# evalf/nutils

Hardware: AMD Instinct MI355X
Metric: elements assembled/sec (global stiffness K) (higher is better)
Workload: dtype f64; 1 GPU; 3D Poisson stiffness, 128^3 structured hex, p=1, 2x2x2 Gauss, iso geometry (BASELINE.json configs[1]); nelems_per_gpu=2097152, nnz_per_gpu=57066625, kernel=k_p1hex_skew<16,16,false,false>, parallelism=single GPU, launch=hipGraph replay (20 steps per graph), settle_steps=600

## Files before the change

nutils_amd/csrc/nh_assemble_p1hex.hip:

```cpp
#include "nh_common.h"
#include <algorithm>
#include <type_traits>
#include <cstdio>
#include <cstdlib>

namespace {

#ifdef NH_ABLATION
#define DEBUG(p) ((p).debug)
#else
#define DEBUG(p) 0
#endif

struct P1Args {
  int n0, n1, n2;
  int lay0, lay1;
  int pl0, pl1;
  const double *verts;
  double origin[3], scale[3];
  double n[2][2];
  double c[3][2];
  double wk[2][2][2];
  double wm[2][2][2];
  int hasm;
  const double *qmass;
  double *values;
  const double *qscale;
  const double *u;
  double *out;
  int accumulate;
  int nbj, nbk;
  long long *tdbg;
  int wbnd;
  int debug;
};

__device__ __forceinline__ int len_of(int X, int N) { return (X > 0) + 1 + (X < N - 1); }
__device__ __forceinline__ i64 cum_of(int X, int N) { return X == 0 ? 0 : 3 * (i64)X - 1; }

__device__ __forceinline__ double fast_rcp(double d) {
  double r = __builtin_amdgcn_rcp(d);
  r = fma(fma(-d, r, 1.), r, r);
  r = fma(fma(-d, r, 1.), r, r);
  return r;
}

__device__ __forceinline__ void lds_barrier() { asm volatile("s_waitcnt lgkmcnt(0)\n\ts_barrier" ::: "memory"); }

struct ElemTables {
  double R0[3][3], R1[3][3], R2[3][3];
  double W01[2][2][3], W02[2][2][3], W12[2][2][3];
  double Mm[3][3][3];
};

__device__ __forceinline__ double element_entry(const ElemTables &T, int a, int bb) {
  const int a0 = a >> 2, a1 = (a >> 1) & 1, a2 = a & 1;
// ... 288 lines not shown
}
__device__ __forceinline__ void half_wait(unsigned *cnt, unsigned target) {
  while (__hip_atomic_load(cnt, __ATOMIC_RELAXED, __HIP_MEMORY_SCOPE_WORKGROUP) < target) __builtin_amdgcn_s_sleep(1);
  asm volatile("" ::: "memory");
}

template <int TJ, int TK, bool MASS, bool COEF>
__global__ __launch_bounds__(2 * TJ * TK) void k_p1hex_skew(P1Args p) {
  constexpr bool VEC = false;
#ifdef NH_ABLATION
  long long tacc[10] = {0, 0, 0, 0, 0, 0, 0, 0, 0, 0}, tprev = clock64();
  const long long tstart = tprev;
  int nslow = 0, nfast = 0;
#ifdef NH_NOTICKS
#define NH_TICK(i)
#else
#define NH_TICK(i) { const long long tnow = clock64(); tacc[i] += tnow - tprev; tprev = tnow; }
#endif
#else
#define NH_TICK(i)
#endif
  constexpr int G = TJ * TK, NT = 2 * G, NP = 4, OJ = TJ - 1, OK = TK - 1, NS = 15, VW = 3;
  constexpr int VJ = TJ + 1, VK = TK + 1, RP = VJ * VK, PS = (RP * NS + 1) & ~1, VPG = (RP + G - 1) / G;
  const bool getenv_stage_late = p.wbnd < 0;
  extern __shared__ __attribute__((aligned(16))) double lds[];
  double *acc = lds;
  double *vbuf = lds + NP * PS;
  unsigned *hcnt = reinterpret_cast<unsigned *>(vbuf + 3 * RP * VW);
  const int tid = threadIdx.x, lt = tid & (G - 1), grp = __builtin_amdgcn_readfirstlane(tid / G);
  const int N0 = p.n0 + 1, N1 = p.n1 + 1, N2 = p.n2 + 1;
  const int NPL = p.pl1 - p.pl0;
  const unsigned wg = gridDim.x % 8 == 0 ? (blockIdx.x % 8) * (gridDim.x / 8) + blockIdx.x / 8 : blockIdx.x;
  const i64 CP = NPL + 2, WI = 16, WB = p.nbj > 1 ? (p.wbnd < 0 ? -p.wbnd : p.wbnd) : 16;
  const i64 rowB = p.nbk * CP * WB, rowI = p.nbk * CP * WI, nmid = max(p.nbj - 2, 0);
  const i64 ctot = (p.nbj > 1 ? 2 : 1) * rowB + nmid * rowI;
  auto unit_at = [&](i64 c) {
    i64 jt, rem, w;
    if (c < rowB) jt = 0, rem = c, w = WB;
    else if (c < rowB + nmid * rowI) jt = 1 + (c - rowB) / rowI, rem = (c - rowB) % rowI, w = WI;
    else jt = p.nbj > 1 ? p.nbj - 1 : 1, rem = c - rowB - nmid * rowI, w = WB;
    const i64 kt = rem / (CP * w), pos = (rem - kt * CP * w) / w;
    return (jt * p.nbk + kt) * NPL + min(max(pos - 1, (i64)0), (i64)NPL);
  };
  i64 u = unit_at(ctot * wg / gridDim.x);
  const i64 u1 = unit_at(ctot * (wg + 1) / gridDim.x);
  if (u >= u1) return;
  auto slot_of = [](int P) { return (int)((unsigned)(P + 2 * NP) % NP) * PS; };
  auto vslot_of = [](int P) { return (int)((unsigned)(P + 3) % 3) * (RP * VW); };
  auto load_vertex = [&](int I, int r, int J0, int K0, double (&x)[3]) {
    const int bb = r / VK, c = r % VK, J = J0 - 1 + bb, K = K0 - 1 + c;
    x[0] = x[1] = x[2] = 0.;
    if (r < RP && I >= 0 && I < N0 && J >= 0 && J < N1 && K >= 0 && K < N2) {
      const double *src = p.verts + (((i64)I * N1 + J) * N2 + K) * 3;
      x[0] = src[0], x[1] = src[1], x[2] = src[2];
    }
  };
  if (tid == 0) *hcnt = 0;
  unsigned htarget = 0;
  const i64 T1 = 3 * (i64)N1 - 2, T2 = 3 * (i64)N2 - 2;
  while (u < u1) {
    const int col = (int)(u / NPL), A = p.pl0 + (int)(u % NPL), B = (int)min((i64)p.pl1, A + (u1 - u));
    const int J0 = (col / p.nbk) * OJ, K0 = (col % p.nbk) * OK;
    {
      constexpr int NVL = (2 * RP + NT - 1) / NT;
      double x[NVL][3];
      bool valid[NVL];
#pragma unroll
      for (int k = 0; k < NVL; ++k) {
        const int v = min(tid + k * NT, 2 * RP - 1), pl = v / RP, r = v % RP, I = A - 1 + pl;
        const int J = J0 - 1 + r / VK, K = K0 - 1 + r % VK;
        valid[k] = I >= 0 && I < N0 && J >= 0 && J < N1 && K >= 0 && K < N2;
        const double *src = p.verts + (((i64)min(max(I, 0), N0 - 1) * N1 + min(max(J, 0), N1 - 1)) * N2 + min(max(K, 0), N2 - 1)) * 3;
        x[k][0] = src[0], x[k][1] = src[1], x[k][2] = src[2];
      }
      for (int t = tid; t < NP * PS / 2; t += NT) reinterpret_cast<double2 *>(acc)[t] = make_double2(0., 0.);
#pragma unroll
      for (int k = 0; k < NVL; ++k) {
        const int v = tid + k * NT, pl = v / RP, r = v % RP;
        if (v < 2 * RP) {
          double *dst = vbuf + vslot_of(A - 1 + pl) + r * VW;
          dst[0] = valid[k] ? x[k][0] : 0., dst[1] = valid[k] ? x[k][1] : 0., dst[2] = valid[k] ? x[k][2] : 0.;
        }
      }
    }
    lds_barrier();

    for (int s = A - 1; s <= B; ++s) {
      htarget += G / 64;
      NH_TICK(0)
      const bool mathrole = ((s - (A - 1)) & 1) == grp;
      if (mathrole) {
        const int ej = lt / TK, ek = lt % TK;
        const int gi = s, gj = J0 - 1 + ej, gk = K0 - 1 + ek;
        if (s < B && gi >= p.lay0 && gi < p.lay1 && gj >= 0 && gj < p.n1 && gk >= 0 && gk < p.n2 && !(DEBUG(p) & 4)) {
#define NH_P1HEX_VERT(a, bb, c) (vbuf + vslot_of(gi + (a)) + ((ej + (bb)) * VK + (ek + (c))) * VW)
#include "nh_p1hex_element.inc"
#undef NH_P1HEX_VERT
        }
        NH_TICK(3)
      } else {
        const bool needv = s + 1 < B && !(DEBUG(p) & 8);
        double Vn[VPG][3];
#pragma unroll
        for (int k = 0; k < VPG; ++k) load_vertex(needv ? s + 2 : -1, lt + k * G, J0, K0, Vn[k]);
        const int P = s - 1;
        bool arrived = false, staged = false;
        auto stage_vertices = [&]() {
#pragma unroll
          for (int k = 0; k < VPG; ++k) {
            const int r = lt + k * G;
            if (r < RP) {
              double *dst = vbuf + vslot_of(s + 2) + r * VW;
              dst[0] = Vn[k][0], dst[1] = Vn[k][1], dst[2] = Vn[k][2];
            }
          }
        };
        if (P >= A && !(DEBUG(p) & 2)) {
          const bool lowJ = J0 == 0, highJ = J0 + OJ >= N1;
          const int cumJ0 = J0 == 0 ? 0 : 3 * J0 - 1;
#ifdef NH_ABLATION
          if (!lowJ && !highJ && P > 0 && P < N0 - 1 && K0 > 0 && K0 + OK < N2) ++nfast; else ++nslow;
#endif
          if (!lowJ && !highJ && P > 0 && P < N0 - 1 && K0 > 0 && K0 + OK < N2) {
            const int e = 2 * lt;
            auto source = [&](int ee, bool &below) {
              const int ok_ = ee / 27, sl_ = ee - ok_ * 27;
              const int dJ_ = (sl_ / 3) % 3 - 1, dK_ = sl_ % 3 - 1;
              below = sl_ < 9;
              return (VK + ok_ + 1) * NS + (sl_ >= 13 ? sl_ - 13 : (dJ_ * VK + dK_) * NS + 13 - sl_);
            };
            bool belowA, belowB;
            const int offA = source(e < 405 ? e : 404, belowA), offB = source(e + 1 < 405 ? e + 1 : 404, belowB);
            const double *sA = acc + (belowA ? slot_of(P - 1) : slot_of(P)) + offA;
            const double *sB = acc + (belowB ? slot_of(P - 1) : slot_of(P)) + offB;
            double a0[OJ], a1[OJ];
#pragma unroll
            for (int i = 0; i < OJ; ++i) {
              a0[i] = sA[i * (VK * NS)];
              a1[i] = sB[i * (VK * NS)];
            }
            const int li = lt - 202;
            const bool lone = li >= 0 && li < OJ;
            bool belowL;
            const int offL = source(404, belowL);
            const double aL = acc[(belowL ? slot_of(P - 1) : slot_of(P)) + offL + (lone ? li : 0) * (VK * NS)];
            half_arrive(hcnt);
            arrived = true;
            NH_TICK(8)
            if (needv && !getenv_stage_late) {
              __builtin_amdgcn_s_waitcnt(0x0f70);
              stage_vertices();
              staged = true;
            }
            const i64 stride8 = 8 * (i64)(9 * (int)T2);
            char *l0 = reinterpret_cast<char *>(p.values + ((3 * (i64)P - 1) * T1 * T2 + 3 * (cumJ0 * T2) + 9 * (3 * (i64)K0 - 1)));
            char *lp = l0 + 16 * lt;
            if (lt < 202) {
#pragma unroll
              for (int i = 0; i < OJ; ++i) {
                if ((DEBUG(p) & 16) && (i & 1)) continue;
                const double2 v = make_double2(a0[i], a1[i]);
                __builtin_memcpy(lp + i * stride8, &v, 16);
              }
            }
            if (lone) *reinterpret_cast<double *>(l0 + li * stride8 + 8 * 404) = aL;
          } else {
            constexpr int RPP = G / 32, KP = (OK + RPP - 1) / RPP;
            const int sl = lt & 31, rsub = lt >> 5;
            const int dI = sl / 9 - 1, dJ = (sl / 3) % 3 - 1, dK = sl % 3 - 1;
            const bool upper = sl >= 13;
            const int need = (dI < 0 ? 1 : dI > 0 ? 8 : 0) | (dJ < 0 ? 2 : dJ > 0 ? 16 : 0) | (dK < 0 ? 4 : dK > 0 ? 32 : 0);
            const int loI = P > 0, hiI = P < N0 - 1, lenI = loI + 1 + hiI;
            double v[KP][OJ];
#pragma unroll
            for (int kp = 0; kp < KP; ++kp) {
              const int ok = kp * RPP + rsub;
              const int srow = (VK + ok + 1) * NS + (upper ? sl - 13 : (dJ * VK + dK) * NS + 13 - sl);
              const double *src = acc + ((!upper && dI < 0) ? slot_of(P - 1) : slot_of(P)) + (ok < OK ? srow : 0);
#pragma unroll
              for (int oj = 0; oj < OJ; ++oj) v[kp][oj] = src[oj * (VK * NS)];
            }
            half_arrive(hcnt);
            arrived = true;
#pragma unroll
            for (int kp = 0; kp < KP; ++kp) {
              const int ok = kp * RPP + rsub, Kk = K0 + ok;
              const bool kact = sl < 27 && ok < OK && Kk < N2;
              const int loK = Kk > 0, hiK = Kk < N2 - 1, lenK = loK + 1 + hiK, cumK = Kk == 0 ? 0 : 3 * Kk - 1;
              double *line = p.values + ((P == 0 ? 0 : 3 * (i64)P - 1) * T1 * T2 + lenI * (cumJ0 * T2));
              if (!lowJ && !highJ) {
                const int flag = loI | 2 | loK << 2 | hiI << 3 | 16 | hiK << 5;
                const unsigned voff8 = 8u * (unsigned)(lenI * 3 * cumK + ((dI + loI) * 3 + (dJ + 1)) * lenK + (dK + loK));
                const i64 stride8 = 8 * (i64)(lenI * 3 * (int)T2);
                if (kact && (flag & need) == need) {
                  char *lp = reinterpret_cast<char *>(line);
#pragma unroll
                  for (int oj = 0; oj < OJ; ++oj) {
                    if (!((DEBUG(p) & 16) && (oj & 1))) *reinterpret_cast<double *>(lp + voff8) = v[kp][oj];
                    lp += stride8;
                  }
                }
              } else {
#pragma unroll
                for (int oj = 0; oj < OJ; ++oj) {
                  const int J = J0 + oj;
                  const int loJ = J > 0, hiJ = J < N1 - 1, lenJ = loJ + 1 + hiJ;
                  const int flag = loI | loJ << 1 | loK << 2 | hiI << 3 | hiJ << 4 | hiK << 5;
                  const unsigned voff = (unsigned)(lenI * lenJ * cumK + ((dI + loI) * lenJ + (dJ + loJ)) * lenK + (dK + loK));
                  if (kact && J < N1 && (flag & need) == need && !((DEBUG(p) & 16) && (oj & 1))) line[voff] = v[kp][oj];
                  line += lenI * lenJ * (int)T2;
                }
              }
            }
          }
        }
        NH_TICK(6)
        if (!arrived) half_arrive(hcnt);
        half_wait(hcnt, htarget);
        NH_TICK(7)
        {
          double2 *z = reinterpret_cast<double2 *>(acc + slot_of(s - 2));
          for (int t = lt; t < PS / 2; t += G) z[t] = make_double2(0., 0.);
        }
        NH_TICK(9)
        if (needv && !staged) stage_vertices();
      }
      if (mathrole) { NH_TICK(1) } else { NH_TICK(4) }
      lds_barrier();
      if (mathrole) { NH_TICK(2) } else { NH_TICK(5) }
    }
    u += B - A;
  }
#ifdef NH_ABLATION
  if (p.tdbg && tid == 0) {
    p.tdbg[16 + 4 * blockIdx.x] = clock64() - tstart;
    p.tdbg[16 + 4 * blockIdx.x + 1] = nfast;
    p.tdbg[16 + 4 * blockIdx.x + 2] = nslow;
  }
  if (p.tdbg && (tid & 63) == 0)
    for (int i = 0; i < 10; ++i) atomicAdd((unsigned long long *)p.tdbg + i, (unsigned long long)tacc[i]);
#endif
}
#undef NH_TICK

__global__ void k_p1hex_unit_matrix(P1Args p, double *Ke) {
  double X[2][2][2][3];
  for (int a = 0; a < 2; ++a)
    for (int b = 0; b < 2; ++b)
      for (int c = 0; c < 2; ++c) {
        X[a][b][c][0] = p.origin[0] + p.scale[0] * a;
        X[a][b][c][1] = p.origin[1] + p.scale[1] * b;
        X[a][b][c][2] = p.origin[2] + p.scale[2] * c;
      }
  ElemTables T;
  {
    double (&R0)[3][3] = T.R0, (&R1)[3][3] = T.R1, (&R2)[3][3] = T.R2;
    double (&W01)[2][2][3] = T.W01, (&W02)[2][2][3] = T.W02, (&W12)[2][2][3] = T.W12;
    double (&Mm)[3][3][3] = T.Mm;
    for (int i = 0; i < 27; ++i) (&Mm[0][0][0])[i] = 0.;
    const bool hasm = p.hasm;
#define NH_P1HEX_QS(q) 1.
#define NH_P1HEX_QM(q) 1.
#include "nh_p1hex_math.inc"
// ... 81 lines not shown
    if (r >= (i64)N0 * N1 * N2) return (3 * (i64)N0 - 2) * T1 * T2;
    const int Kk = (int)(r % N2), J = (int)((r / N2) % N1), I = (int)(r / ((i64)N2 * N1));
    return cum_of(I, N0) * T1 * T2 + len_of(I, N0) * (cum_of(J, N1) * T2 + (i64)len_of(J, N1) * cum_of(Kk, N2));
  };
  const i64 base = rp(row0);
  if (slot == 0) rowptr[row - row0] = rp(row) - base;
  if (row >= row1) return;
  const int Kk = (int)(row % N2), J = (int)((row / N2) % N1), I = (int)(row / ((i64)N2 * N1));
  const int dI = slot / 9 - 1, dJ = (slot / 3) % 3 - 1, dK = slot % 3 - 1;
  const int cI = I + dI, cJ = J + dJ, cK = Kk + dK;
  if (cI < 0 || cI >= N0 || cJ < 0 || cJ >= N1 || cK < 0 || cK >= N2) return;
  const int lenJ = len_of(J, N1), lenK = len_of(Kk, N2);
  const int pos = ((dI + (I > 0)) * lenJ + (dJ + (J > 0))) * lenK + (dK + (Kk > 0));
  colidx[rp(row) - base + pos] = ((i64)cI * N1 + cJ) * N2 + cK;
}

}

template <bool VEC, bool MASS, bool COEF>
static int launch_march_inst(const nh_p1hex_args *a, P1Args &p, void *stream) {
#ifdef NH_ABLATION
  p.debug = getenv("NH_P1HEX_DEBUG") ? atoi(getenv("NH_P1HEX_DEBUG")) : 0;
#endif
  p.wbnd = 20;
#ifdef NH_ABLATION
  static const int wbnd_env = getenv("NH_P1HEX_WBND") ? std::min(64, std::max(8, atoi(getenv("NH_P1HEX_WBND")))) : 20;
  p.wbnd = getenv("NH_P1HEX_STAGE_LATE") ? -wbnd_env : wbnd_env;
#endif
  constexpr int TJ = 16, TK = 16, L = 2, NTM = L * TJ * TK, NS = VEC ? 1 : 15, VW = VEC ? 4 : 3;
  int dev = 0;
  NH_CHECK_HIP(hipGetDevice(&dev));
  NH_REQUIRE(dev >= 0 && dev < 16, "nh_p1hex: device index %d not supported", dev);
  static int cus_of[16] = {0};
  if (!cus_of[dev]) {
    int n = 256;
    NH_CHECK_HIP(hipDeviceGetAttribute(&n, hipDeviceAttributeMultiprocessorCount, dev));
    cus_of[dev] = n;
  }
  const int cus = cus_of[dev];
  p.nbj = (p.n1 + 1 + TJ - 2) / (TJ - 1);
  p.nbk = (p.n2 + 1 + TK - 2) / (TK - 1);
  const size_t ldsm = sizeof(double) * ((L + 2) * (((TJ + 1) * (TK + 1) * NS + 1) & ~1) + (L + 1) * (TJ + 1) * (TK + 1) * VW + 2);
  const i64 units = (i64)p.nbj * p.nbk * (p.pl1 - p.pl0);
  NH_REQUIRE(a->max_workgroups >= 0, "nh_p1hex: negative max_workgroups");
  unsigned grid = (unsigned)std::min<i64>(units, a->max_workgroups ? std::min(cus, a->max_workgroups) : cus);
#ifdef NH_ABLATION
  if (getenv("NH_P1HEX_MAXWG")) grid = std::min<unsigned>(grid, (unsigned)atoi(getenv("NH_P1HEX_MAXWG")));
#endif
  auto kern = k_p1hex_march<TJ, TK, L, VEC, MASS, COEF>;
  if constexpr (!VEC && L == 2) {
    const char *env = getenv("NH_P1HEX_KERNEL");
    if (!(env && !strcmp(env, "march"))) kern = k_p1hex_skew<TJ, TK, MASS, COEF>;
  }
  static const void *attr_set[16][2] = {{nullptr, nullptr}};
  if (attr_set[dev][0] != (const void *)kern && attr_set[dev][1] != (const void *)kern) {
    NH_CHECK_HIP(hipFuncSetAttribute((const void *)kern, hipFuncAttributeMaxDynamicSharedMemorySize, (int)ldsm));
    attr_set[dev][attr_set[dev][0] ? 1 : 0] = (const void *)kern;
  }
#ifdef NH_ABLATION
  static long long *tdbg = nullptr;
  if (!tdbg) NH_CHECK_HIP(hipMalloc((void **)&tdbg, (16 + 4 * 1024) * sizeof(long long)));
  NH_CHECK_HIP(hipMemsetAsync(tdbg, 0, (16 + 4 * 1024) * sizeof(long long), nh_stream(stream)));
  p.tdbg = getenv("NH_P1HEX_TIMERS") ? tdbg : nullptr;
#endif
  hipLaunchKernelGGL(kern, dim3(grid), dim3(NTM), ldsm, nh_stream(stream), p);
  NH_LAUNCH_CHECK();
#ifdef NH_ABLATION
  if (p.tdbg) {
    static long long h[16 + 4 * 1024];
    NH_CHECK_HIP(hipMemcpy(h, tdbg, sizeof h, hipMemcpyDeviceToHost));
    if (getenv("NH_P1HEX_WGTIMES"))
      for (unsigned g = 0; g < grid; ++g) fprintf(stderr, "wg %u cycles %lld fast %lld slow %lld\n", g, h[16 + 4 * g], h[16 + 4 * g + 1], h[16 + 4 * g + 2]);
    const double nw = (double)grid * (NTM / 64);
    if (kern != (void (*)(P1Args))k_p1hex_march<TJ, TK, L, VEC, MASS, COEF>)
      fprintf(stderr, "p1hex_skew cycles per wave: prologue %.0f | math %.0f | - %.0f | math wait %.0f | lds reads %.0f | store issue %.0f | half wait %.0f | zero %.0f | stage %.0f | mem wait %.0f\n", h[0] / nw, h[3] / nw, h[1] / nw,
              h[2] / nw, h[8] / nw, h[6] / nw, h[7] / nw, h[9] / nw, h[4] / nw, h[5] / nw);
    else
    fprintf(stderr, "p1hex_march cycles per wave: stage+next %.0f | B1 %.0f | load+math %.0f | B2 %.0f | stage+flush %.0f | B3 %.0f | zero %.0f\n", h[0] / nw, h[1] / nw,
            h[2] / nw, h[3] / nw, h[4] / nw, h[5] / nw, h[6] / nw);
  }
#endif
  return NH_OK;
}

template <bool VEC>
static int launch_march(const nh_p1hex_args *a, P1Args &p, void *stream) {
  const bool coef = p.qscale || p.qmass;
  if (p.hasm) return coef ? launch_march_inst<VEC, true, true>(a, p, stream) : launch_march_inst<VEC, true, false>(a, p, stream);
  return coef ? launch_march_inst<VEC, false, true>(a, p, stream) : launch_march_inst<VEC, false, false>(a, p, stream);
}

extern "C" {

int nh_p1hex_pattern(const int *shape, int64_t row_begin, int64_t row_end, int64_t *rowptr_dev, int64_t *colidx_dev, void *stream) {
  NH_REQUIRE(shape && rowptr_dev && colidx_dev, "nh_p1hex_pattern: NULL argument");
  NH_REQUIRE(shape[0] >= 1 && shape[1] >= 1 && shape[2] >= 1, "nh_p1hex_pattern: empty mesh");
  const i64 nrows_total = (i64)(shape[0] + 1) * (shape[1] + 1) * (shape[2] + 1);
  NH_REQUIRE(0 <= row_begin && row_begin <= row_end && row_end <= nrows_total, "nh_p1hex_pattern: row range out of bounds");
  const i64 n = (row_end - row_begin + 1) * 27;
  hipLaunchKernelGGL(k_p1hex_pattern, dim3((unsigned)((n + 255) / 256)), dim3(256), 0, nh_stream(stream), shape[0], shape[1], shape[2],
// ... 22 lines not shown
  }
  for (int q = 0; q < 2; ++q) {
    p.n[0][q] = 1. - a->gauss_x[q];
    p.n[1][q] = a->gauss_x[q];
    p.c[0][q] = p.n[0][q] * p.n[0][q];
    p.c[1][q] = p.n[0][q] * p.n[1][q];
    p.c[2][q] = p.n[1][q] * p.n[1][q];
  }
  for (int qa = 0; qa < 2; ++qa)
    for (int qb = 0; qb < 2; ++qb)
      for (int qc = 0; qc < 2; ++qc) {
        p.wk[qa][qb][qc] = a->kappa * a->gauss_w[qa] * a->gauss_w[qb] * a->gauss_w[qc];
        p.wm[qa][qb][qc] = a->mass * a->gauss_w[qa] * a->gauss_w[qb] * a->gauss_w[qc];
      }
  p.hasm = a->mass != 0. || a->qmass_dev != nullptr;
  p.qmass = a->qmass_dev;
  p.values = a->values_dev;
  p.qscale = a->qscale_dev;
  p.u = nullptr;
  p.out = nullptr;
  p.accumulate = 0;
  p.nbj = p.nbk = 0;
  p.debug = 0;
  p.wbnd = 16;
  p.tdbg = nullptr;
  return NH_OK;
}

int nh_p1hex_unit_matrix(const nh_p1hex_args *a, double *ke_dev, void *stream) {
  NH_REQUIRE(ke_dev, "nh_p1hex_unit_matrix: NULL output");
  P1Args p;
  int rc = fill_p1args(a, p);
  if (rc) return rc;
  hipLaunchKernelGGL(k_p1hex_unit_matrix, dim3(1), dim3(1), 0, nh_stream(stream), p, ke_dev);
  NH_LAUNCH_CHECK();
  return NH_OK;
}

int nh_p1hex_laplace(const nh_p1hex_args *a, void *stream) {
  NH_REQUIRE(a && a->values_dev, "nh_p1hex_laplace: NULL argument");
  P1Args p;
  int rc = fill_p1args(a, p);
  if (rc) return rc;
  if (a->plane_begin == a->plane_end) return NH_OK;
  NH_REQUIRE(!(a->qscale_dev || a->qmass_dev) || a->verts_dev, "nh_p1hex_laplace: a coefficient array needs explicit vertices");
  if (!a->verts_dev) {
    double *Ke = nullptr;
// ... 28 lines not shown
```

Before: 12.31 billion elements/s.

## Split workgroups into interior and boundary classes with specialized kernel bodies

Work partitioning now puts boundary column tiles and interior column tiles into separate workgroup classes. Separate weights for the low and high boundary rows and for the corner tiles balance the load between them. The kernel body moves into an include that is instantiated twice. The interior-only version drops the boundary checks and the slow scatter path, and the boundary version adds extra stores for the J-boundary rows. This aims to cut branch and bookkeeping overhead in the common interior case and to improve load balance, at the cost of more code, more register pressure and new host-side split logic.

```diff
diff --git a/nutils_amd/csrc/nh_assemble_p1hex.hip b/nutils_amd/csrc/nh_assemble_p1hex.hip
--- a/nutils_amd/csrc/nh_assemble_p1hex.hip
+++ b/nutils_amd/csrc/nh_assemble_p1hex.hip
@@ -1,4 +1,5 @@
 #include "nh_common.h"
+#include "nh_p1hex_split.h"
 #include <algorithm>
 #include <type_traits>
 #include <cstdio>
@@ -10,6 +11,19 @@
 #define DEBUG(p) ((p).debug)
 #else
 #define DEBUG(p) 0
+#endif
+
+#ifndef NH_P1HEX_WLOW_DEFAULT
+#define NH_P1HEX_WLOW_DEFAULT 19
+#endif
+#ifndef NH_P1HEX_WHIGH_DEFAULT
+#define NH_P1HEX_WHIGH_DEFAULT 18
+#endif
+#ifndef NH_P1HEX_WCLOW_DEFAULT
+#define NH_P1HEX_WCLOW_DEFAULT 22
+#endif
+#ifndef NH_P1HEX_WCHIGH_DEFAULT
+#define NH_P1HEX_WCHIGH_DEFAULT 24
 #endif
 
 struct P1Args {
@@ -31,7 +45,9 @@
   int accumulate;
   int nbj, nbk;
   long long *tdbg;
-  int wbnd;
+  int gb, nfront;
+  int wclow, wchigh;
+  int wlow, whigh;
   int debug;
 };
 
@@ -366,7 +382,7 @@
 #endif
   constexpr int G = TJ * TK, NT = 2 * G, NP = 4, OJ = TJ - 1, OK = TK - 1, NS = 15, VW = 3;
   constexpr int VJ = TJ + 1, VK = TK + 1, RP = VJ * VK, PS = (RP * NS + 1) & ~1, VPG = (RP + G - 1) / G;
-  const bool getenv_stage_late = p.wbnd < 0;
+  const bool getenv_stage_late = p.wlow < 0;
   extern __shared__ __attribute__((aligned(16))) double lds[];
   double *acc = lds;
   double *vbuf = lds + NP * PS;
@@ -375,20 +391,11 @@
   const int N0 = p.n0 + 1, N1 = p.n1 + 1, N2 = p.n2 + 1;
   const int NPL = p.pl1 - p.pl0;
   const unsigned wg = gridDim.x % 8 == 0 ? (blockIdx.x % 8) * (gridDim.x / 8) + blockIdx.x / 8 : blockIdx.x;
-  const i64 CP = NPL + 2, WI = 16, WB = p.nbj > 1 ? (p.wbnd < 0 ? -p.wbnd : p.wbnd) : 16;
-  const i64 rowB = p.nbk * CP * WB, rowI = p.nbk * CP * WI, nmid = max(p.nbj - 2, 0);
-  const i64 ctot = (p.nbj > 1 ? 2 : 1) * rowB + nmid * rowI;
-  auto unit_at = [&](i64 c) {
-    i64 jt, rem, w;
-    if (c < rowB) jt = 0, rem = c, w = WB;
-    else if (c < rowB + nmid * rowI) jt = 1 + (c - rowB) / rowI, rem = (c - rowB) % rowI, w = WI;
-    else jt = p.nbj > 1 ? p.nbj - 1 : 1, rem = c - rowB - nmid * rowI, w = WB;
-    const i64 kt = rem / (CP * w), pos = (rem - kt * CP * w) / w;
-    return (jt * p.nbk + kt) * NPL + min(max(pos - 1, (i64)0), (i64)NPL);
-  };
-  i64 u = unit_at(ctot * wg / gridDim.x);
-  const i64 u1 = unit_at(ctot * (wg + 1) / gridDim.x);
-  if (u >= u1) return;
+  const P1SplitGeom geom = {p.nbj, p.nbk, NPL, p.wlow < 0 ? -p.wlow : p.wlow, p.whigh, p.wclow, p.wchigh};
+  auto uniform = [](i64 x) { return (i64)(((unsigned long long)(unsigned)__builtin_amdgcn_readfirstlane((int)(x >> 32)) << 32) | (unsigned)__builtin_amdgcn_readfirstlane((int)x)); };
+  P1Split sp = nh_p1hex_split_share(geom, gridDim.x, wg, p.gb, p.nfront);
+  sp.cls = __builtin_amdgcn_readfirstlane(sp.cls), sp.v0 = uniform(sp.v0), sp.v1 = uniform(sp.v1);
+  if (sp.v0 >= sp.v1) return;
   auto slot_of = [](int P) { return (int)((unsigned)(P + 2 * NP) % NP) * PS; };
   auto vslot_of = [](int P) { return (int)((unsigned)(P + 3) % 3) * (RP * VW); };
   auto load_vertex = [&](int I, int r, int J0, int K0, double (&x)[3]) {
@@ -402,187 +409,24 @@
   if (tid == 0) *hcnt = 0;
   unsigned htarget = 0;
   const i64 T1 = 3 * (i64)N1 - 2, T2 = 3 * (i64)N2 - 2;
-  while (u < u1) {
-    const int col = (int)(u / NPL), A = p.pl0 + (int)(u % NPL), B = (int)min((i64)p.pl1, A + (u1 - u));
-    const int J0 = (col / p.nbk) * OJ, K0 = (col % p.nbk) * OK;
-    {
-      constexpr int NVL = (2 * RP + NT - 1) / NT;
-      double x[NVL][3];
-      bool valid[NVL];
-#pragma unroll
-      for (int k = 0; k < NVL; ++k) {
-        const int v = min(tid + k * NT, 2 * RP - 1), pl = v / RP, r = v % RP, I = A - 1 + pl;
-        const int J = J0 - 1 + r / VK, K = K0 - 1 + r % VK;
-        valid[k] = I >= 0 && I < N0 && J >= 0 && J < N1 && K >= 0 && K < N2;
-        const double *src = p.verts + (((i64)min(max(I, 0), N0 - 1) * N1 + min(max(J, 0), N1 - 1)) * N2 + min(max(K, 0), N2 - 1)) * 3;
-        x[k][0] = src[0], x[k][1] = src[1], x[k][2] = src[2];
-      }
-      for (int t = tid; t < NP * PS / 2; t += NT) reinterpret_cast<double2 *>(acc)[t] = make_double2(0., 0.);
-#pragma unroll
-      for (int k = 0; k < NVL; ++k) {
-        const int v = tid + k * NT, pl = v / RP, r = v % RP;
-        if (v < 2 * RP) {
-          double *dst = vbuf + vslot_of(A - 1 + pl) + r * VW;
-          dst[0] = valid[k] ? x[k][0] : 0., dst[1] = valid[k] ? x[k][1] : 0., dst[2] = valid[k] ? x[k][2] : 0.;
-        }
-      }
-    }
-    lds_barrier();
-
-    for (int s = A - 1; s <= B; ++s) {
-      htarget += G / 64;
-      NH_TICK(0)
-      const bool mathrole = ((s - (A - 1)) & 1) == grp;
-      if (mathrole) {
-        const int ej = lt / TK, ek = lt % TK;
-        const int gi = s, gj = J0 - 1 + ej, gk = K0 - 1 + ek;
-        if (s < B && gi >= p.lay0 && gi < p.lay1 && gj >= 0 && gj < p.n1 && gk >= 0 && gk < p.n2 && !(DEBUG(p) & 4)) {
-#define NH_P1HEX_VERT(a, bb, c) (vbuf + vslot_of(gi + (a)) + ((ej + (bb)) * VK + (ek + (c))) * VW)
-#include "nh_p1hex_element.inc"
-#undef NH_P1HEX_VERT
-        }
-        NH_TICK(3)
-      } else {
-        const bool needv = s + 1 < B && !(DEBUG(p) & 8);
-        double Vn[VPG][3];
-#pragma unroll
-        for (int k = 0; k < VPG; ++k) load_vertex(needv ? s + 2 : -1, lt + k * G, J0, K0, Vn[k]);
-        const int P = s - 1;
-        bool arrived = false, staged = false;
-        auto stage_vertices = [&]() {
-#pragma unroll
-          for (int k = 0; k < VPG; ++k) {
-            const int r = lt + k * G;
-            if (r < RP) {
-              double *dst = vbuf + vslot_of(s + 2) + r * VW;
-              dst[0] = Vn[k][0], dst[1] = Vn[k][1], dst[2] = Vn[k][2];
-            }
-          }
-        };
-        if (P >= A && !(DEBUG(p) & 2)) {
-          const bool lowJ = J0 == 0, highJ = J0 + OJ >= N1;
-          const int cumJ0 = J0 == 0 ? 0 : 3 * J0 - 1;
-#ifdef NH_ABLATION
-          if (!lowJ && !highJ && P > 0 && P < N0 - 1 && K0 > 0 && K0 + OK < N2) ++nfast; else ++nslow;
-#endif
-          if (!lowJ && !highJ && P > 0 && P < N0 - 1 && K0 > 0 && K0 + OK < N2) {
-            const int e = 2 * lt;
-            auto source = [&](int ee, bool &below) {
-              const int ok_ = ee / 27, sl_ = ee - ok_ * 27;
-              const int dJ_ = (sl_ / 3) % 3 - 1, dK_ = sl_ % 3 - 1;
-              below = sl_ < 9;
-              return (VK + ok_ + 1) * NS + (sl_ >= 13 ? sl_ - 13 : (dJ_ * VK + dK_) * NS + 13 - sl_);
-            };
-            bool belowA, belowB;
-            const int offA = source(e < 405 ? e : 404, belowA), offB = source(e + 1 < 405 ? e + 1 : 404, belowB);
-            const double *sA = acc + (belowA ? slot_of(P - 1) : slot_of(P)) + offA;
-            const double *sB = acc + (belowB ? slot_of(P - 1) : slot_of(P)) + offB;
-            double a0[OJ], a1[OJ];
-#pragma unroll
-            for (int i = 0; i < OJ; ++i) {
-              a0[i] = sA[i * (VK * NS)];
-              a1[i] = sB[i * (VK * NS)];
-            }
-            const int li = lt - 202;
-            const bool lone = li >= 0 && li < OJ;
-            bool belowL;
-            const int offL = source(404, belowL);
-            const double aL = acc[(belowL ? slot_of(P - 1) : slot_of(P)) + offL + (lone ? li : 0) * (VK * NS)];
-            half_arrive(hcnt);
-            arrived = true;
-            NH_TICK(8)
-            if (needv && !getenv_stage_late) {
-              __builtin_amdgcn_s_waitcnt(0x0f70);
-              stage_vertices();
-              staged = true;
-            }
-            const i64 stride8 = 8 * (i64)(9 * (int)T2);
-            char *l0 = reinterpret_cast<char *>(p.values + ((3 * (i64)P - 1) * T1 * T2 + 3 * (cumJ0 * T2) + 9 * (3 * (i64)K0 - 1)));
-            char *lp = l0 + 16 * lt;
-            if (lt < 202) {
-#pragma unroll
-              for (int i = 0; i < OJ; ++i) {
-                if ((DEBUG(p) & 16) && (i & 1)) continue;
-                const double2 v = make_double2(a0[i], a1[i]);
-                __builtin_memcpy(lp + i * stride8, &v, 16);
-              }
-            }
-            if (lone) *reinterpret_cast<double *>(l0 + li * stride8 + 8 * 404) = aL;
-          } else {
-            constexpr int RPP = G / 32, KP = (OK + RPP - 1) / RPP;
-            const int sl = lt & 31, rsub = lt >> 5;
-            const int dI = sl / 9 - 1, dJ = (sl / 3) % 3 - 1, dK = sl % 3 - 1;
-            const bool upper = sl >= 13;
-            const int need = (dI < 0 ? 1 : dI > 0 ? 8 : 0) | (dJ < 0 ? 2 : dJ > 0 ? 16 : 0) | (dK < 0 ? 4 : dK > 0 ? 32 : 0);
-            const int loI = P > 0, hiI = P < N0 - 1, lenI = loI + 1 + hiI;
-            double v[KP][OJ];
-#pragma unroll
-            for (int kp = 0; kp < KP; ++kp) {
-              const int ok = kp * RPP + rsub;
-              const int srow = (VK + ok + 1) * NS + (upper ? sl - 13 : (dJ * VK + dK) * NS + 13 - sl);
-              const double *src = acc + ((!upper && dI < 0) ? slot_of(P - 1) : slot_of(P)) + (ok < OK ? srow : 0);
-#pragma unroll
-              for (int oj = 0; oj < OJ; ++oj) v[kp][oj] = src[oj * (VK * NS)];
-            }
-            half_arrive(hcnt);
-            arrived = true;
-#pragma unroll
-            for (int kp = 0; kp < KP; ++kp) {
-              const int ok = kp * RPP + rsub, Kk = K0 + ok;
-              const bool kact = sl < 27 && ok < OK && Kk < N2;
-              const int loK = Kk > 0, hiK = Kk < N2 - 1, lenK = loK + 1 + hiK, cumK = Kk == 0 ? 0 : 3 * Kk - 1;
-              double *line = p.values + ((P == 0 ? 0 : 3 * (i64)P - 1) * T1 * T2 + lenI * (cumJ0 * T2));
-              if (!lowJ && !highJ) {
-                const int flag = loI | 2 | loK << 2 | hiI << 3 | 16 | hiK << 5;
-                const unsigned voff8 = 8u * (unsigned)(lenI * 3 * cumK + ((dI + loI) * 3 + (dJ + 1)) * lenK + (dK + loK));
-                const i64 stride8 = 8 * (i64)(lenI * 3 * (int)T2);
-                if (kact && (flag & need) == need) {
-                  char *lp = reinterpret_cast<char *>(line);
-#pragma unroll
-                  for (int oj = 0; oj < OJ; ++oj) {
-                    if (!((DEBUG(p) & 16) && (oj & 1))) *reinterpret_cast<double *>(lp + voff8) = v[kp][oj];
-                    lp += stride8;
-                  }
-                }
-              } else {
-#pragma unroll
-                for (int oj = 0; oj < OJ; ++oj) {
-                  const int J = J0 + oj;
-                  const int loJ = J > 0, hiJ = J < N1 - 1, lenJ = loJ + 1 + hiJ;
-                  const int flag = loI | loJ << 1 | loK << 2 | hiI << 3 | hiJ << 4 | hiK << 5;
-                  const unsigned voff = (unsigned)(lenI * lenJ * cumK + ((dI + loI) * lenJ + (dJ + loJ)) * lenK + (dK + loK));
-                  if (kact && J < N1 && (flag & need) == need && !((DEBUG(p) & 16) && (oj & 1))) line[voff] = v[kp][oj];
-                  line += lenI * lenJ * (int)T2;
-                }
-              }
-            }
-          }
-        }
-        NH_TICK(6)
-        if (!arrived) half_arrive(hcnt);
-        half_wait(hcnt, htarget);
-        NH_TICK(7)
-        {
-          double2 *z = reinterpret_cast<double2 *>(acc + slot_of(s - 2));
-          for (int t = lt; t < PS / 2; t += G) z[t] = make_double2(0., 0.);
-        }
-        NH_TICK(9)
-        if (needv && !staged) stage_vertices();
-      }
-      if (mathrole) { NH_TICK(1) } else { NH_TICK(4) }
-      lds_barrier();
-      if (mathrole) { NH_TICK(2) } else { NH_TICK(5) }
-    }
-    u += B - A;
+  if (!MASS && !COEF && sp.cls == NH_P1_INTERIOR) {
+#define NH_P1HEX_BND false
+#include "nh_p1hex_skew_run.inc"
+#undef NH_P1HEX_BND
+  } else {
+#define NH_P1HEX_BND true
+#include "nh_p1hex_skew_run.inc"
+#undef NH_P1HEX_BND
   }
 #ifdef NH_ABLATION
   if (p.tdbg && tid == 0) {
-    p.tdbg[16 + 4 * blockIdx.x] = clock64() - tstart;
-    p.tdbg[16 + 4 * blockIdx.x + 1] = nfast;
-    p.tdbg[16 + 4 * blockIdx.x + 2] = nslow;
+    p.tdbg[32 + 4 * blockIdx.x] = clock64() - tstart;
+    p.tdbg[32 + 4 * blockIdx.x + 1] = nfast;
+    p.tdbg[32 + 4 * blockIdx.x + 2] = nslow;
+    p.tdbg[32 + 4 * blockIdx.x + 3] = sp.cls;
   }
   if (p.tdbg && (tid & 63) == 0)
-    for (int i = 0; i < 10; ++i) atomicAdd((unsigned long long *)p.tdbg + i, (unsigned long long)tacc[i]);
+    for (int i = 0; i < 10; ++i) atomicAdd((unsigned long long *)p.tdbg + (sp.cls == NH_P1_INTERIOR ? 0 : 10) + i, (unsigned long long)tacc[i]);
 #endif
 }
 #undef NH_TICK
@@ -710,10 +554,16 @@
 #ifdef NH_ABLATION
   p.debug = getenv("NH_P1HEX_DEBUG") ? atoi(getenv("NH_P1HEX_DEBUG")) : 0;
 #endif
-  p.wbnd = 20;
-#ifdef NH_ABLATION
-  static const int wbnd_env = getenv("NH_P1HEX_WBND") ? std::min(64, std::max(8, atoi(getenv("NH_P1HEX_WBND")))) : 20;
-  p.wbnd = getenv("NH_P1HEX_STAGE_LATE") ? -wbnd_env : wbnd_env;
+  p.wlow = NH_P1HEX_WLOW_DEFAULT;
+  p.whigh = NH_P1HEX_WHIGH_DEFAULT;
+  p.wclow = NH_P1HEX_WCLOW_DEFAULT;
+  p.wchigh = NH_P1HEX_WCHIGH_DEFAULT;
+#ifdef NH_ABLATION
+  if (getenv("NH_P1HEX_WLOW")) p.wlow = std::min(64, std::max(8, atoi(getenv("NH_P1HEX_WLOW"))));
+  if (getenv("NH_P1HEX_WHIGH")) p.whigh = std::min(64, std::max(8, atoi(getenv("NH_P1HEX_WHIGH"))));
+  if (getenv("NH_P1HEX_WCLOW")) p.wclow = std::min(64, std::max(8, atoi(getenv("NH_P1HEX_WCLOW"))));
+  if (getenv("NH_P1HEX_WCHIGH")) p.wchigh = std::min(64, std::max(8, atoi(getenv("NH_P1HEX_WCHIGH"))));
+  if (getenv("NH_P1HEX_STAGE_LATE")) p.wlow = -p.wlow;
 #endif
   constexpr int TJ = 16, TK = 16, L = 2, NTM = L * TJ * TK, NS = VEC ? 1 : 15, VW = VEC ? 4 : 3;
   int dev = 0;
@@ -747,23 +597,47 @@
   }
 #ifdef NH_ABLATION
   static long long *tdbg = nullptr;
-  if (!tdbg) NH_CHECK_HIP(hipMalloc((void **)&tdbg, (16 + 4 * 1024) * sizeof(long long)));
-  NH_CHECK_HIP(hipMemsetAsync(tdbg, 0, (16 + 4 * 1024) * sizeof(long long), nh_stream(stream)));
+  if (!tdbg) NH_CHECK_HIP(hipMalloc((void **)&tdbg, (32 + 4 * 1024) * sizeof(long long)));
+  NH_CHECK_HIP(hipMemsetAsync(tdbg, 0, (32 + 4 * 1024) * sizeof(long long), nh_stream(stream)));
   p.tdbg = getenv("NH_P1HEX_TIMERS") ? tdbg : nullptr;
 #endif
+  {
+    const P1SplitGeom geom = {p.nbj, p.nbk, p.pl1 - p.pl0, p.wlow < 0 ? -p.wlow : p.wlow, p.whigh, p.wclow, p.wchigh};
+    const P1SplitClasses c = nh_p1hex_split_classes(geom, grid);
+    p.gb = (int)c.gb, p.nfront = (int)c.nfront;
+  }
   hipLaunchKernelGGL(kern, dim3(grid), dim3(NTM), ldsm, nh_stream(stream), p);
   NH_LAUNCH_CHECK();
 #ifdef NH_ABLATION
   if (p.tdbg) {
-    static long long h[16 + 4 * 1024];
+    static long long h[32 + 4 * 1024];
     NH_CHECK_HIP(hipMemcpy(h, tdbg, sizeof h, hipMemcpyDeviceToHost));
-    if (getenv("NH_P1HEX_WGTIMES"))
-      for (unsigned g = 0; g < grid; ++g) fprintf(stderr, "wg %u cycles %lld fast %lld slow %lld\n", g, h[16 + 4 * g], h[16 + 4 * g + 1], h[16 + 4 * g + 2]);
     const double nw = (double)grid * (NTM / 64);
-    if (kern != (void (*)(P1Args))k_p1hex_march<TJ, TK, L, VEC, MASS, COEF>)
-      fprintf(stderr, "p1hex_skew cycles per wave: prologue %.0f | math %.0f | - %.0f | math wait %.0f | lds reads %.0f | store issue %.0f | half wait %.0f | zero %.0f | stage %.0f | mem wait %.0f\n", h[0] / nw, h[3] / nw, h[1] / nw,
-              h[2] / nw, h[8] / nw, h[6] / nw, h[7] / nw, h[9] / nw, h[4] / nw, h[5] / nw);
-    else
+    if (kern != (void (*)(P1Args))k_p1hex_march<TJ, TK, L, VEC, MASS, COEF>) {
+      static const char *const cname[3] = {"interior", "boundary", "mixed"};
+      double cnt[3] = {0, 0, 0}, sum[3] = {0, 0, 0}, lo[3] = {0, 0, 0}, hi[3] = {0, 0, 0};
+      for (unsigned g = 0; g < grid; ++g) {
+        const long long cyc = h[32 + 4 * g], c = std::min(2ll, std::max(0ll, h[32 + 4 * g + 3]));
+        if (!cyc) continue;
+        if (getenv("NH_P1HEX_WGTIMES")) {
+          const P1SplitGeom geom = {p.nbj, p.nbk, p.pl1 - p.pl0, p.wlow < 0 ? -p.wlow : p.wlow, p.whigh, p.wclow, p.wchigh};
+          const unsigned share = grid % 8 == 0 ? (g % 8) * (grid / 8) + g / 8 : g;
+          const P1Split s = nh_p1hex_split(geom, grid, share);
+          const long long col = nh_p1hex_class_column(geom, s.cls, s.v0 / geom.npl);
+          fprintf(stderr, "wg %u share %u class %s first column jt %lld kt %lld units %lld cycles %lld fast %lld slow %lld\n", g, share, cname[c], col / p.nbk, col % p.nbk, s.v1 - s.v0, cyc,
+                  h[32 + 4 * g + 1], h[32 + 4 * g + 2]);
+        }
+        lo[c] = cnt[c] ? std::min(lo[c], (double)cyc) : (double)cyc, hi[c] = std::max(hi[c], (double)cyc), sum[c] += cyc, cnt[c] += 1;
+      }
+      for (int c = 0; c < 3; ++c)
+        if (cnt[c]) fprintf(stderr, "p1hex_skew class %s: %.0f workgroups, cycles mean %.0f min %.0f max %.0f\n", cname[c], cnt[c], sum[c] / cnt[c], lo[c], hi[c]);
+      for (int b = 0; b < 2; ++b) {
+        const double nwb = (b ? cnt[1] + cnt[2] : cnt[0]) * (NTM / 64);
+        const long long *t = h + 10 * b;
+        if (nwb) fprintf(stderr, "p1hex_skew %s body, cycles per wave: prologue %.0f | math %.0f | - %.0f | math wait %.0f | lds reads %.0f | store issue %.0f | half wait %.0f | zero %.0f | stage %.0f | mem wait %.0f\n",
+                         b ? "boundary" : "interior", t[0] / nwb, t[3] / nwb, t[1] / nwb, t[2] / nwb, t[8] / nwb, t[6] / nwb, t[7] / nwb, t[9] / nwb, t[4] / nwb, t[5] / nwb);
+      }
+    } else
     fprintf(stderr, "p1hex_march cycles per wave: stage+next %.0f | B1 %.0f | load+math %.0f | B2 %.0f | stage+flush %.0f | B3 %.0f | zero %.0f\n", h[0] / nw, h[1] / nw,
             h[2] / nw, h[3] / nw, h[4] / nw, h[5] / nw, h[6] / nw);
   }
@@ -832,7 +706,8 @@
   p.accumulate = 0;
   p.nbj = p.nbk = 0;
   p.debug = 0;
-  p.wbnd = 16;
+  p.wlow = p.whigh = p.wclow = p.wchigh = 16;
+  p.gb = p.nfront = 0;
   p.tdbg = nullptr;
   return NH_OK;
 }
diff --git a/nutils_amd/csrc/nh_p1hex_skew_run.inc b/nutils_amd/csrc/nh_p1hex_skew_run.inc
--- /dev/null
+++ b/nutils_amd/csrc/nh_p1hex_skew_run.inc
@@ -0,0 +1,212 @@
+{
+  constexpr bool BND = NH_P1HEX_BND;
+  int tid_ = tid, lt_ = lt;
+  asm volatile("" : "+v"(tid_), "+v"(lt_));
+  {
+  const int tid = tid_ & (NT - 1), lt = lt_ & (G - 1);
+  i64 u = sp.v0;
+  const i64 u1 = sp.v1;
+  while (u < u1) {
+    const int col = __builtin_amdgcn_readfirstlane((int)nh_p1hex_class_column(geom, BND ? sp.cls : NH_P1_INTERIOR, u / NPL)), A = __builtin_amdgcn_readfirstlane(p.pl0 + (int)(u % NPL));
+    const int B = (int)min((i64)p.pl1, A + (u1 - u));
+    const int J0 = (col / p.nbk) * OJ, K0 = (col % p.nbk) * OK;
+    {
+      constexpr int NVL = (2 * RP + NT - 1) / NT;
+      double x[NVL][3];
+      bool valid[NVL];
+#pragma unroll
+      for (int k = 0; k < NVL; ++k) {
+        const int v = min(tid + k * NT, 2 * RP - 1), pl = v / RP, r = v % RP, I = A - 1 + pl;
+        const int J = J0 - 1 + r / VK, K = K0 - 1 + r % VK;
+        valid[k] = I >= 0 && I < N0 && J >= 0 && J < N1 && K >= 0 && K < N2;
+        const double *src = p.verts + (((i64)min(max(I, 0), N0 - 1) * N1 + min(max(J, 0), N1 - 1)) * N2 + min(max(K, 0), N2 - 1)) * 3;
+        x[k][0] = src[0], x[k][1] = src[1], x[k][2] = src[2];
+      }
+      for (int t = tid; t < NP * PS / 2; t += NT) reinterpret_cast<double2 *>(acc)[t] = make_double2(0., 0.);
+#pragma unroll
+      for (int k = 0; k < NVL; ++k) {
+        const int v = tid + k * NT, pl = v / RP, r = v % RP;
+        if (v < 2 * RP) {
+          double *dst = vbuf + vslot_of(A - 1 + pl) + r * VW;
+          dst[0] = valid[k] ? x[k][0] : 0., dst[1] = valid[k] ? x[k][1] : 0., dst[2] = valid[k] ? x[k][2] : 0.;
+        }
+      }
+    }
+    lds_barrier();
+
+    for (int s = A - 1; s <= B; ++s) {
+      htarget += G / 64;
+      NH_TICK(0)
+      const bool mathrole = ((s - (A - 1)) & 1) == grp;
+      if (mathrole) {
+        const int ej = lt / TK, ek = lt % TK;
+        const int gi = s, gj = J0 - 1 + ej, gk = K0 - 1 + ek;
+        if (s < B && gi >= p.lay0 && gi < p.lay1 && gj >= 0 && gj < p.n1 && gk >= 0 && gk < p.n2 && !(DEBUG(p) & 4)) {
+#define NH_P1HEX_VERT(a, bb, c) (vbuf + vslot_of(gi + (a)) + ((ej + (bb)) * VK + (ek + (c))) * VW)
+#include "nh_p1hex_element.inc"
+#undef NH_P1HEX_VERT
+        }
+        NH_TICK(3)
+      } else {
+        const bool needv = s + 1 < B && !(DEBUG(p) & 8);
+        double Vn[VPG][3];
+#pragma unroll
+        for (int k = 0; k < VPG; ++k) load_vertex(needv ? s + 2 : -1, lt + k * G, J0, K0, Vn[k]);
+        const int P = s - 1;
+        bool arrived = false, staged = false;
+        auto stage_vertices = [&]() {
+#pragma unroll
+          for (int k = 0; k < VPG; ++k) {
+            const int r = lt + k * G;
+            if (r < RP) {
+              double *dst = vbuf + vslot_of(s + 2) + r * VW;
+              dst[0] = Vn[k][0], dst[1] = Vn[k][1], dst[2] = Vn[k][2];
+            }
+          }
+        };
+        if (P >= A && !(DEBUG(p) & 2)) {
+          const bool lowJ = BND && J0 == 0, highJ = BND && J0 + OJ >= N1;
+          const int cumJ0 = 3 * J0 - 1;
+          const bool linewise = !(lowJ && highJ) && P > 0 && P < N0 - 1 && K0 > 0 && K0 + OK < N2;
+#ifdef NH_ABLATION
+          if (linewise) ++nfast; else ++nslow;
+#endif
+          if (linewise) {
+            const int jlo = lowJ ? 1 : 0, jhi = highJ ? N1 - 1 - J0 : OJ;
+            const int e = 2 * lt;
+            auto source = [&](int ee, bool &below) {
+              const int ok_ = ee / 27, sl_ = ee - ok_ * 27;
+              const int dJ_ = (sl_ / 3) % 3 - 1, dK_ = sl_ % 3 - 1;
+              below = sl_ < 9;
+              return (VK + ok_ + 1) * NS + (sl_ >= 13 ? sl_ - 13 : (dJ_ * VK + dK_) * NS + 13 - sl_);
+            };
+            bool belowA, belowB;
+            const int offA = source(e < 405 ? e : 404, belowA), offB = source(e + 1 < 405 ? e + 1 : 404, belowB);
+            const double *sA = acc + (belowA ? slot_of(P - 1) : slot_of(P)) + offA;
+            const double *sB = acc + (belowB ? slot_of(P - 1) : slot_of(P)) + offB;
+            double a0[OJ], a1[OJ];
+#pragma unroll
+            for (int i = 0; i < OJ; ++i) {
+              if (!BND || (i >= jlo && i < jhi)) {
+                a0[i] = sA[i * (VK * NS)];
+                a1[i] = sB[i * (VK * NS)];
+              } else a0[i] = a1[i] = 0.;
+            }
+            const int li = lt - 202;
+            const bool lone = li >= jlo && li < jhi;
+            bool belowL;
+            const int offL = source(404, belowL);
+            const double aL = acc[(belowL ? slot_of(P - 1) : slot_of(P)) + offL + (lone ? li : jlo < jhi ? jlo : 0) * (VK * NS)];
+            double b0 = 0., b1 = 0.;
+            if (BND && (lowJ || highJ) && lt < 135) {
+              int e = 2 * lt;
+              asm volatile("" : "+v"(e));
+              const int jb = lowJ ? 0 : N1 - 1 - J0;
+              auto source18 = [&](int ee, bool &below) {
+                const int ok_ = ee / 18, s_ = ee - ok_ * 18;
+                const int dJ_ = (s_ / 3) % 2 - (lowJ ? 0 : 1), dK_ = s_ % 3 - 1, sl_ = (s_ / 6) * 9 + (dJ_ + 1) * 3 + (dK_ + 1);
+                below = sl_ < 9;
+                return (VK + ok_ + 1) * NS + (sl_ >= 13 ? sl_ - 13 : (dJ_ * VK + dK_) * NS + 13 - sl_);
+              };
+              bool belowC, belowD;
+              const int offC = source18(e, belowC) + jb * (VK * NS), offD = source18(e + 1, belowD) + jb * (VK * NS);
+              b0 = acc[(belowC ? slot_of(P - 1) : slot_of(P)) + offC];
+              b1 = acc[(belowD ? slot_of(P - 1) : slot_of(P)) + offD];
+            }
+            half_arrive(hcnt);
+            arrived = true;
+            NH_TICK(8)
+            if (needv && !getenv_stage_late) {
+              __builtin_amdgcn_s_waitcnt(0x0f70);
+              stage_vertices();
+              staged = true;
+            }
+            const i64 stride8 = 8 * (i64)(9 * (int)T2);
+            char *const pbase = reinterpret_cast<char *>(p.values + (3 * (i64)P - 1) * T1 * T2);
+            char *l0 = pbase + 8 * (3 * (cumJ0 * T2) + 9 * (3 * (i64)K0 - 1));
+            char *lp = l0 + 16 * lt;
+            if (lt < 202) {
+#pragma unroll
+              for (int i = 0; i < OJ; ++i) {
+                if ((DEBUG(p) & 16) && (i & 1)) continue;
+                if (BND && !(i >= jlo && i < jhi)) continue;
+                const double2 v = make_double2(a0[i], a1[i]);
+                __builtin_memcpy(lp + i * stride8, &v, 16);
+              }
+            }
+            if (lone) *reinterpret_cast<double *>(l0 + li * stride8 + 8 * 404) = aL;
+            if (BND && (lowJ || highJ) && lt < 135) {
+              const i64 cumJb = lowJ ? 0 : 3 * (i64)(N1 - 1) - 1;
+              const double2 v = make_double2(b0, b1);
+              __builtin_memcpy(pbase + 8 * (3 * (cumJb * T2) + 6 * (3 * (i64)K0 - 1)) + 16 * lt, &v, 16);
+            }
+          } else {
+            constexpr int RPP = G / 32, KP = (OK + RPP - 1) / RPP;
+            const int sl = lt & 31, rsub = lt >> 5;
+            const int dI = sl / 9 - 1, dJ = (sl / 3) % 3 - 1, dK = sl % 3 - 1;
+            const bool upper = sl >= 13;
+            const int need = (dI < 0 ? 1 : dI > 0 ? 8 : 0) | (dJ < 0 ? 2 : dJ > 0 ? 16 : 0) | (dK < 0 ? 4 : dK > 0 ? 32 : 0);
+            const int loI = P > 0, hiI = P < N0 - 1, lenI = loI + 1 + hiI;
+            const int cumJ0g = J0 == 0 ? 0 : cumJ0;
+            double v[KP][OJ];
+#pragma unroll
+            for (int kp = 0; kp < KP; ++kp) {
+              const int ok = kp * RPP + rsub;
+              const int srow = (VK + ok + 1) * NS + (upper ? sl - 13 : (dJ * VK + dK) * NS + 13 - sl);
+              const double *src = acc + ((!upper && dI < 0) ? slot_of(P - 1) : slot_of(P)) + (ok < OK ? srow : 0);
+#pragma unroll
+              for (int oj = 0; oj < OJ; ++oj) v[kp][oj] = src[oj * (VK * NS)];
+            }
+            half_arrive(hcnt);
+            arrived = true;
+#pragma unroll
+            for (int kp = 0; kp < KP; ++kp) {
+              const int ok = kp * RPP + rsub, Kk = K0 + ok;
+              const bool kact = sl < 27 && ok < OK && Kk < N2;
+              const int loK = Kk > 0, hiK = Kk < N2 - 1, lenK = loK + 1 + hiK, cumK = Kk == 0 ? 0 : 3 * Kk - 1;
+              double *line = p.values + ((P == 0 ? 0 : 3 * (i64)P - 1) * T1 * T2 + lenI * (cumJ0g * T2));
+              if (!lowJ && !highJ) {
+                const int flag = loI | 2 | loK << 2 | hiI << 3 | 16 | hiK << 5;
+                const unsigned voff8 = 8u * (unsigned)(lenI * 3 * cumK + ((dI + loI) * 3 + (dJ + 1)) * lenK + (dK + loK));
+                const i64 stride8 = 8 * (i64)(lenI * 3 * (int)T2);
+                if (kact && (flag & need) == need) {
+                  char *lp = reinterpret_cast<char *>(line);
+#pragma unroll
+                  for (int oj = 0; oj < OJ; ++oj) {
+                    if (!((DEBUG(p) & 16) && (oj & 1))) *reinterpret_cast<double *>(lp + voff8) = v[kp][oj];
+                    lp += stride8;
+                  }
+                }
+              } else {
+#pragma unroll
+                for (int oj = 0; oj < OJ; ++oj) {
+                  const int J = J0 + oj;
+                  const int loJ = J > 0, hiJ = J < N1 - 1, lenJ = loJ + 1 + hiJ;
+                  const int flag = loI | loJ << 1 | loK << 2 | hiI << 3 | hiJ << 4 | hiK << 5;
+                  const unsigned voff = (unsigned)(lenI * lenJ * cumK + ((dI + loI) * lenJ + (dJ + loJ)) * lenK + (dK + loK));
+                  if (kact && J < N1 && (flag & need) == need && !((DEBUG(p) & 16) && (oj & 1))) line[voff] = v[kp][oj];
+                  line += lenI * lenJ * (int)T2;
+                }
+              }
+            }
+          }
+        }
+        NH_TICK(6)
+        if (!arrived) half_arrive(hcnt);
+        half_wait(hcnt, htarget);
+        NH_TICK(7)
+        {
+          double2 *z = reinterpret_cast<double2 *>(acc + slot_of(s - 2));
+          for (int t = lt; t < PS / 2; t += G) z[t] = make_double2(0., 0.);
+        }
+        NH_TICK(9)
+        if (needv && !staged) stage_vertices();
+      }
+      if (mathrole) { NH_TICK(1) } else { NH_TICK(4) }
+      lds_barrier();
+      if (mathrole) { NH_TICK(2) } else { NH_TICK(5) }
+    }
+    u += B - A;
+  }
+  }
+}
diff --git a/nutils_amd/csrc/nh_p1hex_split.h b/nutils_amd/csrc/nh_p1hex_split.h
--- /dev/null
+++ b/nutils_amd/csrc/nh_p1hex_split.h
@@ -0,0 +1,107 @@
+#ifndef NH_P1HEX_SPLIT_H
+#define NH_P1HEX_SPLIT_H
+
+#if defined(__HIPCC__)
+#define NH_SPLIT_FN __host__ __device__ __attribute__((always_inline)) inline
+#else
+#define NH_SPLIT_FN inline
+#endif
+
+enum { NH_P1_INTERIOR = 0, NH_P1_BOUNDARY = 1, NH_P1_MIXED = 2 };
+
+struct P1SplitGeom {
+  int nbj, nbk;
+  int npl;
+  int wlow, whigh;
+  int wclow, wchigh;
+};
+
+struct P1Split {
+  int cls;
+  long long v0, v1;
+};
+
+struct P1SplitAxis {
+  long long na, wa, wca, nb, wb, wcb, nc, wc, wcc;
+};
+
+NH_SPLIT_FN P1SplitAxis nh_p1hex_axis(const P1SplitGeom &g, int cls) {
+  const long long nmid = g.nbj > 2 ? (long long)(g.nbj - 2) * g.nbk : 0, nhigh = g.nbj > 1 ? g.nbk : 0;
+  P1SplitAxis a;
+  a.na = cls == NH_P1_INTERIOR ? 0 : g.nbk, a.wa = g.wlow, a.wca = g.wclow;
+  a.nb = cls == NH_P1_BOUNDARY ? 0 : nmid, a.wb = 16, a.wcb = 16;
+  a.nc = cls == NH_P1_INTERIOR ? 0 : nhigh, a.wc = g.whigh, a.wcc = g.wchigh;
+  return a;
+}
+
+NH_SPLIT_FN long long nh_p1hex_block_weight(long long n, long long w, long long wc) { return n <= 0 ? 0 : n == 1 ? wc : 2 * wc + (n - 2) * w; }
+
+NH_SPLIT_FN long long nh_p1hex_axis_cost(const P1SplitGeom &g, const P1SplitAxis &a) {
+  return (nh_p1hex_block_weight(a.na, a.wa, a.wca) + nh_p1hex_block_weight(a.nb, a.wb, a.wcb) + nh_p1hex_block_weight(a.nc, a.wc, a.wcc)) * (g.npl + 2);
+}
+
+NH_SPLIT_FN long long nh_p1hex_axis_unit(const P1SplitGeom &g, const P1SplitAxis &a, long long c) {
+  const long long CP = g.npl + 2;
+  const long long la = nh_p1hex_block_weight(a.na, a.wa, a.wca) * CP, lb = nh_p1hex_block_weight(a.nb, a.wb, a.wcb) * CP, lc = nh_p1hex_block_weight(a.nc, a.wc, a.wcc) * CP;
+  if (c >= la + lb + lc) return (a.na + a.nb + a.nc) * g.npl;
+  const bool ina = c < la, inb = !ina && c < la + lb;
+  long long rem = ina ? c : inb ? c - la : c - la - lb;
+  const long long n = ina ? a.na : inb ? a.nb : a.nc, w = ina ? a.wa : inb ? a.wb : a.wc, wc = ina ? a.wca : inb ? a.wcb : a.wcc;
+  const long long col0 = ina ? 0 : inb ? a.na : a.na + a.nb;
+  long long kt = 0, ww = wc;
+  if (rem >= CP * wc) {
+    rem -= CP * wc;
+    const long long nm = n > 2 ? n - 2 : 0;
+    if (rem < nm * CP * w) kt = rem / (CP * w), rem -= kt * CP * w, kt += 1, ww = w;
+    else rem -= nm * CP * w, kt = nm + 1;
+  }
+  const long long pl = rem / ww - 1;
+  return (col0 + kt) * g.npl + (pl < 0 ? 0 : pl > g.npl ? g.npl : pl);
+}
+
+NH_SPLIT_FN long long nh_p1hex_class_column(const P1SplitGeom &g, int cls, long long lc) {
+  if (cls == NH_P1_INTERIOR) return lc + g.nbk;
+  if (cls == NH_P1_BOUNDARY && lc >= g.nbk) return lc + (long long)(g.nbj - 2) * g.nbk;
+  return lc;
+}
+
+struct P1SplitClasses {
+  long long gb, nfront;
+};
+
+NH_SPLIT_FN P1SplitClasses nh_p1hex_split_classes(const P1SplitGeom &g, long long grid) {
+  const P1SplitAxis ab = nh_p1hex_axis(g, NH_P1_BOUNDARY), ai = nh_p1hex_axis(g, NH_P1_INTERIOR);
+  const long long cb = nh_p1hex_axis_cost(g, ab), ci = nh_p1hex_axis_cost(g, ai);
+  P1SplitClasses c;
+  c.gb = c.nfront = grid;
+  if (ci > 0 && grid < 2) c.gb = -1;
+  else if (ci > 0) {
+    c.gb = (grid * cb + (cb + ci) / 2) / (cb + ci);
+    c.gb = c.gb < 1 ? 1 : c.gb > grid - 1 ? grid - 1 : c.gb;
+    c.nfront = (c.gb * nh_p1hex_block_weight(ab.na, ab.wa, ab.wca) * (g.npl + 2) + cb / 2) / cb;
+    c.nfront = c.nfront > c.gb ? c.gb : c.nfront;
+  }
+  return c;
+}
+
+NH_SPLIT_FN P1Split nh_p1hex_split_share(const P1SplitGeom &g, long long grid, long long wg, long long gb, long long nfront) {
+  P1Split s;
+  long long n = grid, i = wg;
+  s.cls = NH_P1_BOUNDARY;
+  if (gb < 0) s.cls = NH_P1_MIXED;
+  else if (wg < nfront) n = gb;
+  else if (wg >= grid - (gb - nfront)) n = gb, i = wg - (grid - gb);
+  else s.cls = NH_P1_INTERIOR, n = grid - gb, i = wg - nfront;
+  const P1SplitAxis a = nh_p1hex_axis(g, s.cls);
+  const long long cost = nh_p1hex_axis_cost(g, a);
+  s.v0 = nh_p1hex_axis_unit(g, a, cost * i / n);
+  s.v1 = nh_p1hex_axis_unit(g, a, cost * (i + 1) / n);
+  return s;
+}
+
+NH_SPLIT_FN P1Split nh_p1hex_split(const P1SplitGeom &g, long long grid, long long wg) {
+  const P1SplitClasses c = nh_p1hex_split_classes(g, grid);
+  return nh_p1hex_split_share(g, grid, wg, c.gb, c.nfront);
+}
+
+#endif
```

Result: no change. 12.31 billion elements/s (-0.0%).
